# ratt-ru/pfb-clean

Hardware: AMD Instinct MI355X
Metric: PCG matvecs/sec (FFT-conv A^H A apply), 4k x 4k x 8-band cube (higher is better)
Workload: dtype f32; 1 GPU; 4096x4096x8-band cube PCG (hessian_psf + Tikhonov, M = x/sigmainv, tol=0, minit=maxit=20); nx_psf=8192, bands_per_gpu=8, parallelism=band-shard x1, allreduce_hook=False

## Files before the change

pfb_clean_amd/csrc/fftconv_pow2.hip:

```cpp
#include "conv_plan.hpp"
#include "fft_pow2.hpp"
#include <vector>
#include <cstdlib>
#include <type_traits>

namespace pfb {

#ifndef PFB_STAMP
#define PFB_STAMP 0
#endif
#if PFB_STAMP
#define PFB_STAMP_ITS 4
#define PFB_STAMP_FIRST 2
static __device__ unsigned long long* g_stamp_buf = nullptr;
#define STAMP(KID, it, slot)                                                                              \
    do {                                                                                                  \
        const unsigned _si = (unsigned)((it) - PFB_STAMP_FIRST);                                          \
        if (threadIdx.x == 0 && g_stamp_buf && _si < PFB_STAMP_ITS && blockIdx.x < 1024)                  \
            g_stamp_buf[(((size_t)(KID) * 1024 + blockIdx.x) * PFB_STAMP_ITS + _si) * 16 + (slot)] = wall_clock64(); \
    } while (0)
#else
#define STAMP(KID, it, slot) do { (void)(it); } while (0)
#endif

// ... 787 lines not shown
    if constexpr (K < NREG) {
        hook(PassIdx<K>{});
        Blk<T, NVB> o;
#pragma unroll
        for (int h = 0; h < NVB; ++h) {
            cplx<T> w;
            if constexpr (P::BIG) w = K == 0 ? lw[h] : lw[h] * root32<T>(P::KR * K);
            else w = lw[MS * K + h];
            if (PAR) w = w * wq1;
            const cplx<T> zv = za[h][F::cpad(MS * K)];
            cplx<T> zm = zb[h][F::cpad(MS * (NREG - 1 - K))];
            if constexpr (PAR == 0 && K == 0) { if (first0 && h == 0) zm = zv; }
            o.c[h] = T(0.5) * addrot<false>(addc(zv, zm), w * subc(zv, zm));
        }
        storeb<T, NVB>(ub + (size_t)K * ustep + voff, o);
        __builtin_amdgcn_sched_barrier(0);
        post_steps_lin<T, L, PAR, K + 1, NREG, Hook>(za, zb, lw, wq1, ub, ustep, voff, first0, hook);
    }
}

template <typename T, int L, int PAR, typename Hook = NoPassHook>
__device__ __forceinline__ void fwdp_post(const cplx<T>* zr, const cplx<T>* ltm, cplx<T> wq1,
                                          cplx<T>* __restrict__ Tb, int nx, int i0, int rr, int bi,
                                          const Hook& hook = Hook()) {
    using P = FwdP<T, L>;
    using F = typename P::F;
    constexpr int NVB = P::NVB, BS = P::BSTEP, MS = NVB * BS;
    constexpr int NBP = PAR ? P::NBO : P::NBE;
    constexpr int NIT = (NBP + BS - 1) / BS;
    constexpr int NREG = PAR ? NIT : NIT - 1;
    static_assert(MS % 16 == 0, "a step keeps the padding phase");
    static_assert(PAR ? (NBP == NIT * BS) : (NBP == (NIT - 1) * BS + 1), "block counts of the two sweeps");
    cplx<T>* ub = Tb + (size_t)(PAR ? P::NBE : 0) * nx * NVB;
    const size_t ustep = (size_t)BS * nx * NVB;
    const unsigned voff = ((unsigned)bi * (unsigned)nx + (unsigned)(i0 + rr)) * NVB;
    const int m0 = NVB * bi;
    const cplx<T>* za[NVB];
    const cplx<T>* zb[NVB];
#pragma unroll
    for (int h = 0; h < NVB; ++h) {
        za[h] = zr + F::pad(m0 + h);
        zb[h] = zr + F::pad(L - PAR - (m0 + h) - MS * (NREG - 1));
    }
    post_steps_lin<T, L, PAR, 0, NREG, Hook>(za, zb, ltm + m0, wq1, ub, ustep, voff, bi == 0, hook);
    if constexpr (PAR == 0) {
        hook(PassIdx<NREG>{});
        const cplx<T> z0 = zr[F::pad(0)];
        Blk<T, NVB> o;
        o.c[0] = T(0.5) * addrot<false>(addc(z0, z0), cplx<T>(T(-1), T(0)) * subc(z0, z0));
#pragma unroll
        for (int h = 1; h < NVB; ++h) o.c[h] = cplx<T>(0, 0);
        storeb<T, NVB>(ub + (size_t)(NBP - 1) * nx * NVB + (unsigned)(i0 + rr) * NVB, o);
        __builtin_amdgcn_sched_barrier(0);
    }
}

template <typename T, int L, bool BEAM>
__global__ void __launch_bounds__((FwdP<T, L>::NT))
k_row_fwd_pow2q(const T* __restrict__ x, const T* __restrict__ beam, cplx<T>* __restrict__ Tw, const cplx<T>* __restrict__ twM,
                const cplx<T>* __restrict__ ptwc, FastDims d, int band0, int tiles_per_band, int ntiles,
                cplx<T> wq1) {
    using P = FwdP<T, L>;
    constexpr int E = P::E;
    using F = RegFft<T, L, E, false, 0, true, false>;
    constexpr int TPB = F::TPB, G = P::G, NT = P::NT, NP = F::NPASS;
    using V2 = typename vec2<T>::type;
    extern __shared__ __attribute__((aligned(16))) char smem[];
    cplx<T>* ltw = reinterpret_cast<cplx<T>*>(smem);
    cplx<T>* ltm = ltw + P::PTWP;
    cplx<T>* lds0 = ltm + P::NTM;
    int vb = blockIdx.x;
    if (vb >= ntiles) return;
    for (int k = threadIdx.x; k < F::PTWC; k += NT) ltw[k] = ptwc[k];
    for (int k = threadIdx.x; k < P::NTM; k += NT) ltm[k] = twM[k];
    V2 xa[E], ba[BEAM ? E : 1];
    {
        const int bl = vb / tiles_per_band, i0 = P::tile_row(vb - bl * tiles_per_band, tiles_per_band);
        const int g = threadIdx.x / TPB, t = threadIdx.x % TPB;
        const size_t off = (size_t)bl * d.xband + (size_t)(i0 + g) * d.xpitch;
        const V2* xr = reinterpret_cast<const V2*>(x + off) + t;
#pragma unroll
        for (int j = 0; j < E; ++j) xa[j] = xr[TPB * j];
        if constexpr (BEAM) {
            const V2* br = reinterpret_cast<const V2*>(beam + off) + t;
#pragma unroll
            for (int j = 0; j < E; ++j) ba[j] = br[TPB * j];
        }
    }
    __syncthreads();
    for (int sit = 0;; ++sit) {
        STAMP(0, sit, 0);
        const int vbn = vb + (int)gridDim.x < ntiles ? vb + (int)gridDim.x : vb;
        const int bl = vb / tiles_per_band, i0 = P::tile_row(vb - bl * tiles_per_band, tiles_per_band);
        cplx<T>* Tb = Tw + (size_t)(band0 + bl) * d.T_band;
        cplx<T> vv[E];
        {
            const int tid = launder((int)threadIdx.x);
            const int g = tid / TPB, t = tid % TPB;
            cplx<T>* lds = lds0 + (size_t)g * P::STRIDE;
#pragma unroll
            for (int j = 0; j < E; ++j) {
                if constexpr (BEAM) { xa[j].x *= ba[j].x; xa[j].y *= ba[j].y; }
                vv[j] = cplx<T>(xa[j].x, xa[j].y);
            }
            STAMP(0, sit, 1);
            F::template run<false>(vv, lds, t, ltw);
            STAMP(0, sit, 2);
        }
        {
            const int tid = launder((int)threadIdx.x);
            const int g = tid / TPB, t = tid % TPB;
            __syncthreads();
            cplx<T>* wp = lds0 + (size_t)g * P::STRIDE + F::pad(t);
#pragma unroll
            for (int j = 0; j < E; ++j) wp[F::cpad(TPB * j)] = vv[j];
            __syncthreads();
        }
        STAMP(0, sit, 3);
        {
            const int tid = launder((int)threadIdx.x);
            fwdp_post<T, L, 0>(lds0 + (size_t)(tid % G) * P::STRIDE, ltm, wq1, Tb, d.nx, i0, tid % G, tid / G);
        }
        STAMP(0, sit, 4);
        {
            const int tid = launder((int)threadIdx.x);
            const int g = tid / TPB, t = tid % TPB;
            cplx<T>* lds = lds0 + (size_t)g * P::STRIDE;
#pragma unroll
            for (int j = 0; j < E; ++j) {
                vv[j] = cplx<T>(xa[j].x, xa[j].y) * P::tw_row(ltm, t, j);
                if ((j & 3) == 3) __builtin_amdgcn_sched_barrier(0);
            }
            const int bln = vbn / tiles_per_band, i0n = P::tile_row(vbn - bln * tiles_per_band, tiles_per_band);
            const size_t offn = (size_t)bln * d.xband + (size_t)(i0n + g) * d.xpitch;
            const V2* xr = reinterpret_cast<const V2*>(x + offn) + t;
            const V2* br = BEAM ? reinterpret_cast<const V2*>(beam + offn) + t : nullptr;
            F::template run<false>(vv, lds, t, ltw, [&](auto k) {
                constexpr int K = decltype(k)::value;
#pragma unroll
                for (int j = (K * E) / NP; j < ((K + 1) * E) / NP; ++j) {
                    xa[j] = xr[TPB * j];
                    if constexpr (BEAM) ba[j] = br[TPB * j];
                }
            });
            STAMP(0, sit, 5);
        }
        {
            const int tid = launder((int)threadIdx.x);
            const int g = tid / TPB, t = tid % TPB;
            cplx<T>* wp = lds0 + (size_t)g * P::STRIDE + F::pad(t);
            __syncthreads();
#pragma unroll
            for (int j = 0; j < E; ++j) wp[F::cpad(TPB * j)] = vv[j];
            __syncthreads();
            fwdp_post<T, L, 1>(lds0 + (size_t)(tid % G) * P::STRIDE, ltm, wq1, Tb, d.nx, i0, tid % G, tid / G);
            STAMP(0, sit, 6);
            __syncthreads();
        }
        STAMP(0, sit, 7);
        if (vbn == vb) break;
        vb = vbn;
    }
}

template <typename T, int L, int E, int PAR, typename PF>
__device__ __forceinline__ void row_inv_phase(PF&& after_loads_issued, const cplx<T>* __restrict__ Tb,
                                              const cplx<T>* __restrict__ twQ,
                                              const cplx<T>* __restrict__ ptw, cplx<T>* lds0,
                                              cplx<T>* lds, int nx, int i0, int t,
                                              cplx<T> (&vv)[E]) {
    using F = RegFft<T, L, E, RowCfg<T, L, true>::WAVE, InvDb<T, L>::OFF, true>;
    constexpr int TPB = F::TPB;
    constexpr int G = row_groups<T, L, E, RowCfg<T, L, true>::GMAX>();
    constexpr int NT = G * TPB;
    constexpr int STRIDE = F::LDS_ELEMS + 4;
    const int rr = threadIdx.x % G, bi = threadIdx.x / G;
    cplx<T>* yr = lds0 + (size_t)rr * STRIDE;
    __syncthreads();
    constexpr int NVB = FastCfg<T>::NVB;
    constexpr int NBE = nblocks_even(L, NVB);
    constexpr int NBP = PAR ? nblocks_odd(L, NVB) : NBE;
    constexpr int BSTEP = NT / G;
    const cplx<T>* Tp = Tb + ((size_t)(PAR ? NBE : 0) * nx + i0 + rr) * NVB;
    constexpr int NIT = (NBP + BSTEP - 1) / BSTEP;
    Blk<T, NVB> y[NIT];
#pragma unroll
    for (int k = 0; k < NIT; ++k) {
        const int b = bi + k * BSTEP;
        if (b < NBP) y[k] = loadb<T, NVB>(Tp + (size_t)b * nx * NVB);
    }
    after_loads_issued();
#pragma unroll
    for (int k = 0; k < NIT; ++k) {
        const int b = bi + k * BSTEP;
        if (b < NBP) {
#pragma unroll
            for (int h = 0; h < NVB; ++h)
                if (PAR || NVB * b + h <= L) yr[F::pad(NVB * b + h)] = y[k].c[h];
        }
    }
    __syncthreads();
#pragma unroll
    for (int j = 0; j < E; ++j) {
        const int m = t + TPB * j;
        cplx<T> yv = lds[F::pad(m)];
        cplx<T> ym = lds[F::pad(PAR ? (L - 1 - m) : (L - m))];
        if (!PAR && m == 0) { yv.y = 0; ym.y = 0; }
        const cplx<T> w = twQ[2 * m + PAR];
        vv[j] = addrot<true>(addc(yv, ym), mulc(subc(yv, ym), w));
        if ((j & 3) == 3) __builtin_amdgcn_sched_barrier(0);
    }
    F::template run<true>(vv, lds, t, ptw);
}

template <typename T, int L, int E>
__global__ void __launch_bounds__((row_groups<T, L, E, RowCfg<T, L, true>::GMAX>() * (L / E)))
k_row_inv_pow2(const cplx<T>* __restrict__ Tw, const cplx<T>* __restrict__ twQ,
               const cplx<T>* __restrict__ twM, const cplx<T>* __restrict__ ptw,
               const T* __restrict__ x, const T* __restrict__ beam,
               const T* __restrict__ dot_with, const T* __restrict__ dot_with2, T* __restrict__ out,
               double* __restrict__ partials, FastDims d, int band0, T scale, T sigmainv) {
    using F = RegFft<T, L, E, RowCfg<T, L, true>::WAVE, InvDb<T, L>::OFF, true>;
    constexpr int TPB = F::TPB;
    constexpr int G = row_groups<T, L, E, RowCfg<T, L, true>::GMAX>();
    constexpr int NT = G * TPB;
    constexpr int STRIDE = F::LDS_ELEMS + 4;
    constexpr int HP = G / 2;
    using V2 = typename vec2<T>::type;
    extern __shared__ __attribute__((aligned(16))) char smem[];
    double* red = reinterpret_cast<double*>(smem);
    cplx<T>* ltw = reinterpret_cast<cplx<T>*>(smem + 384);
    cplx<T>* lds0 = ltw + ((F::PTWC + 1) & ~1);
    const int g = threadIdx.x / TPB, t = threadIdx.x % TPB;
    cplx<T>* lds = lds0 + (size_t)g * STRIDE;
    for (int k = threadIdx.x; k < F::PTWC; k += NT) ltw[k] = ptw[k];
    const int rg = xcd_row_group<G>(blockIdx.x, gridDim.x);
    const int i0 = rg * G;
    const int bl = blockIdx.y, band = band0 + bl;
    const cplx<T>* Tb = Tw + (size_t)band * d.T_band;
    cplx<T> vv[E], ev[E];
    row_inv_phase<T, L, E, 0>([] {}, Tb, twQ, ltw, lds0, lds, d.nx, i0, t, ev);
    const size_t rowoff = ((size_t)bl * d.nx + (i0 + g)) * d.ny;
    const V2* xr = reinterpret_cast<const V2*>(x + rowoff) + t;
    const V2* br = beam ? reinterpret_cast<const V2*>(beam + rowoff) + t : nullptr;
    const V2* dr = dot_with ? reinterpret_cast<const V2*>(dot_with + rowoff) + t : nullptr;
    const V2* dr2 = dot_with2 ? reinterpret_cast<const V2*>(dot_with2 + rowoff) + t : nullptr;
    V2* orow = reinterpret_cast<V2*>(out + rowoff) + t;
    const bool dot_is_x = dot_with == x;
    constexpr bool BIG32 = sizeof(T) == 4 && E >= 16 && L >= 4096;
    constexpr bool MIXBIG = odd_part(L) > 1 && (NT >= 1024 || E >= 16 || (sizeof(T) == 8 && NT >= 512));
    constexpr bool PREF = !BIG32 && !MIXBIG && (sizeof(T) == 4 || NT < 1024);
    V2 xq[PREF ? E : 1], rq[PREF ? E : 1];
    row_inv_phase<T, L, E, 1>([&] {
        if constexpr (PREF) {
#pragma unroll
            for (int j = 0; j < E; ++j) {
                xq[j] = xr[TPB * j];
                if (dr2) rq[j] = dr2[TPB * j];
            }
        }
    }, Tb, twQ, ltw, lds0, lds, d.nx, i0, t, vv);
    double acc[3] = {0.0, 0.0, 0.0};
    const cplx<T>* tm = twM + t;
#pragma unroll
    for (int j = 0; j < E; ++j) {
        const cplx<T> zz = ev[j] + mulc(vv[j], tm[TPB * j]);
        V2 val;
        val.x = zz.x * scale;
        val.y = zz.y * scale;
        if (br) { const V2 b = br[TPB * j]; val.x *= b.x; val.y *= b.y; }
        V2 xx;
        if constexpr (PREF) xx = xq[j]; else xx = xr[TPB * j];
        val.x += sigmainv * xx.x;
        val.y += sigmainv * xx.y;
        orow[TPB * j] = val;
        if (dr) {
            V2 dw = xx;
            if (!dot_is_x) dw = dr[TPB * j];
            acc[0] += (double)dw.x * (double)val.x + (double)dw.y * (double)val.y;
            if (dr2) {
                V2 d2;
                if constexpr (PREF) d2 = rq[j]; else d2 = dr2[TPB * j];
                acc[1] += (double)d2.x * (double)val.x + (double)d2.y * (double)val.y;
            }
            acc[2] += (double)val.x * (double)val.x + (double)val.y * (double)val.y;
        }
    }
    if (dot_with) {
        __syncthreads();
        block_sum<3>(acc, red);
        if (threadIdx.x == 0) {
            const size_t np = (size_t)gridDim.x * gridDim.y, k = (size_t)bl * gridDim.x + rg;
            partials[k] = acc[0]; partials[np + k] = acc[1]; partials[2 * np + k] = acc[2];
        }
    }
}

constexpr int INV_ROT = 3;
constexpr int INV_HOIST_B = 8;
template <typename T, int L, int E>
struct InvP {
    using C = RowCfg<T, L, true>;
    using F = RegFft<T, L, E, C::WAVE, 0, true>;
    static constexpr bool PARK = sizeof(T) == 4 && E < 16;
    static constexpr int G = (sizeof(T) == 4 ? 1024 : 512) / F::TPB;
    static constexpr int NT = G * F::TPB;
    static constexpr int STRIDE = F::LDS_ELEMS + 4;
    static constexpr int NVB = FastCfg<T>::NVB;
    static constexpr int NBE = nblocks_even(L, NVB);
    static constexpr int NBO = nblocks_odd(L, NVB);
    static constexpr int BSTEP = NT / G;
    static constexpr int NITE = (NBE + BSTEP - 1) / BSTEP;
    static constexpr int NITO = (NBO + BSTEP - 1) / BSTEP;
    static constexpr int PTWP = (F::PTWC + 1) & ~1;
    static constexpr bool SMT = E >= 16;
    static constexpr bool OPF = E < 16;
    static constexpr bool NXT = OPF || sizeof(T) == 8;
    static constexpr bool NXE = !NXT;
    static constexpr int NTM = SMT ? F::TPB : L;
    static constexpr size_t LDS = 384 + sizeof(cplx<T>) * ((size_t)PTWP + NTM + (size_t)G * STRIDE + (PARK ? (size_t)G * L : 0));
    static constexpr bool OK = odd_part(L) == 1 && LDS <= (size_t)LDS_MAX && !C::WAVE && (!SMT || 32 * F::TPB == 2 * L) &&
                               (sizeof(T) == 4 ? (NT == 1024 && G >= 4 && G <= 16) : (NT == 512 && (G == 2 || G == 4) && L >= 1024));
    __device__ __forceinline__ static cplx<T> tw_row(const cplx<T>* ltm, int t, int j) {
        if constexpr (SMT) return j == 0 ? ltm[t] : ltm[t] * root32<T>(j);
        else return ltm[t + F::TPB * j];
    }
};

template <typename T, int L> struct InvPE {
    static constexpr int MINL64 = 4096;
    static constexpr int E = (sizeof(T) == 8 && L >= MINL64) ? 16 : RowCfg<T, L, true>::E;
};

template <typename T, int L>
constexpr bool invp_class(int e, bool park, bool opf, bool smt, bool nxt) {
    using P = InvP<T, L, InvPE<T, L>::E>;
    return P::OK && InvPE<T, L>::E == e && P::PARK == park && P::OPF == opf && P::SMT == smt && P::NXT == nxt &&
           P::NXE == !nxt && P::SMT == !opf && (nxt || sizeof(T) == 4);
}
static_assert(invp_class<float, 1024>(8, true, true, false, true) && invp_class<float, 2048>(8, true, true, false, true));
static_assert(invp_class<double, 1024>(8, false, true, false, true) && invp_class<double, 2048>(8, false, true, false, true));
static_assert(invp_class<double, 4096>(16, false, false, true, true) && invp_class<float, 4096>(16, false, false, true, false));

template <typename T, int L, int E>
constexpr bool inv_pb_ok() { return odd_part(L) == 1 && !(sizeof(T) == 4 && InvP<T, L, E>::SMT); }

template <typename T, int L, int E>
constexpr bool inv_lin_ok() {
    using P = InvP<T, L, E>;
    return sizeof(T) == 4 && P::NBO % P::BSTEP == 0 && P::NBE == P::NBO + 1 && P::NITO * P::BSTEP == P::NBO &&
           P::NITE == P::NITO + 1 && (P::NVB * P::BSTEP) % 16 == 0 && P::F::TPB % 16 == 0;
}
template <typename T, int L, int E, int PAR, int K0, int K1>
__device__ __forceinline__ void inv_issue_slice(const cplx<T>* __restrict__ Tb, int nx, int i0, int rr, int bi,
                                                Blk<T, FastCfg<T>::NVB> (&y)[InvP<T, L, E>::NITE]);
template <typename T, int L, int E, int PAR>
__device__ __forceinline__ void inv_issue(const cplx<T>* __restrict__ Tb, int nx, int i0, int rr, int bi,
                                          Blk<T, FastCfg<T>::NVB> (&y)[InvP<T, L, E>::NITE]) {
    using P = InvP<T, L, E>;
    constexpr int NBP = PAR ? P::NBO : P::NBE, NIT = PAR ? P::NITO : P::NITE;
    if constexpr (inv_lin_ok<T, L, E>()) {
        inv_issue_slice<T, L, E, PAR, 0, NIT>(Tb, nx, i0, rr, bi, y);
        return;
    }
    const cplx<T>* Tp = Tb + ((size_t)(PAR ? P::NBE : 0) * nx + i0 + rr) * P::NVB;
#pragma unroll
    for (int k = 0; k < NIT; ++k) {
        int b = bi + k * P::BSTEP;
        if (b >= NBP) b = NBP - 1;
        y[k] = loadb<T, P::NVB>(Tp + (size_t)b * nx * P::NVB);
    }
}

template <typename T, int L, int E, int PAR, int K0, int K1>
__device__ __forceinline__ void inv_issue_slice(const cplx<T>* __restrict__ Tb, int nx, int i0, int rr, int bi,
                                                Blk<T, FastCfg<T>::NVB> (&y)[InvP<T, L, E>::NITE]) {
    using P = InvP<T, L, E>;
    constexpr int NBP = PAR ? P::NBO : P::NBE;
    if constexpr (inv_lin_ok<T, L, E>()) {
        const cplx<T>* ub = Tb + (size_t)(PAR ? P::NBE : 0) * nx * P::NVB;
        const size_t ustep = (size_t)P::BSTEP * nx * P::NVB;
        const unsigned vrow = (unsigned)(i0 + rr) * P::NVB, voff = (unsigned)bi * (unsigned)nx * P::NVB + vrow;
#pragma unroll
        for (int k = K0; k < K1; ++k) {
            if (PAR == 0 && k == P::NITE - 1) y[k] = loadb<T, P::NVB>(ub + (size_t)(NBP - 1) * nx * P::NVB + vrow);
            else y[k] = loadb<T, P::NVB>(ub + (size_t)k * ustep + voff);
        }
        return;
    }
    const cplx<T>* Tp = Tb + ((size_t)(PAR ? P::NBE : 0) * nx + i0 + rr) * P::NVB;
#pragma unroll
    for (int k = K0; k < K1; ++k) {
        int b = bi + k * P::BSTEP;
        if (b >= NBP) b = NBP - 1;
        y[k] = loadb<T, P::NVB>(Tp + (size_t)b * nx * P::NVB);
    }
}

template <typename T, int L, int E, int PAR>
__device__ __forceinline__ void inv_scatter(const Blk<T, FastCfg<T>::NVB> (&y)[InvP<T, L, E>::NITE],
                                            cplx<T>* yr, int bi) {
    using P = InvP<T, L, E>;
    constexpr int NBP = PAR ? P::NBO : P::NBE, NIT = PAR ? P::NITO : P::NITE;
    if constexpr (inv_lin_ok<T, L, E>()) {
        cplx<T>* y0 = yr + P::F::pad(P::NVB * bi);
#pragma unroll
        for (int k = 0; k < NIT; ++k) {
            if (PAR == 0 && k == NIT - 1) yr[P::F::pad(L)] = y[k].c[0];
            else {
#pragma unroll
                for (int h = 0; h < P::NVB; ++h) y0[P::F::cpad(P::NVB * P::BSTEP * k) + h] = y[k].c[h];
            }
        }
        return;
    }
#pragma unroll
    for (int k = 0; k < NIT; ++k) {
        int b = bi + k * P::BSTEP;
        if (b >= NBP) b = NBP - 1;
#pragma unroll
        for (int h = 0; h < P::NVB; ++h)
            if (PAR || P::NVB * b + h <= L) yr[P::F::pad(P::NVB * b + h)] = y[k].c[h];
    }
}

template <typename T, int L, int E, int PAR>
__device__ __forceinline__ void inv_build(const cplx<T>* lds, const cplx<T>* ltm, cplx<T> wq1, int t,
                                          cplx<T> (&vv)[E]) {
    using F = typename InvP<T, L, E>::F;
    if constexpr (inv_lin_ok<T, L, E>()) {
        const cplx<T>* pa = lds + F::pad(t);
        const cplx<T>* pb = lds + F::pad(L - PAR - t - F::TPB * (E - 1));
#pragma unroll
        for (int j = 0; j < E; ++j) {
            cplx<T> yv = pa[F::cpad(F::TPB * j)];
            cplx<T> ym = pb[F::cpad(F::TPB * (E - 1 - j))];
            if (!PAR && j == 0) { if (t == 0) { yv.y = 0; ym.y = 0; } }
            cplx<T> w = InvP<T, L, E>::tw_row(ltm, t, j);
            if (PAR) w = w * wq1;
            vv[j] = addrot<true>(addc(yv, ym), mulc(subc(yv, ym), w));
            if ((j & 3) == 3) __builtin_amdgcn_sched_barrier(0);
        }
        return;
    }
#pragma unroll
    for (int j = 0; j < E; ++j) {
        const int m = t + F::TPB * j;
        cplx<T> yv = lds[F::pad(m)];
        cplx<T> ym = lds[F::pad(PAR ? (L - 1 - m) : (L - m))];
        if (!PAR && m == 0) { yv.y = 0; ym.y = 0; }
        cplx<T> w = InvP<T, L, E>::tw_row(ltm, t, j);
        if (PAR) w = w * wq1;
        vv[j] = addrot<true>(addc(yv, ym), mulc(subc(yv, ym), w));
        if ((j & 3) == 3) __builtin_amdgcn_sched_barrier(0);
    }
}

template <typename T, int L, int E, int MODE, bool BEAM, bool PB = false>
__global__ void __launch_bounds__((InvP<T, L, E>::NT), (InvP<T, L, E>::NT / 256))
k_row_inv_pow2p(const cplx<T>* __restrict__ Tw, const cplx<T>* __restrict__ twM,
                const cplx<T>* __restrict__ ptw, const T* __restrict__ x, const T* __restrict__ beam,
                const T* __restrict__ dot_with2, T* __restrict__ out,
                double* __restrict__ partials, FastDims d, int band0, int tiles_per_band, int ntiles,
                T scale, T sigmainv, cplx<T> wq1) {
    using P = InvP<T, L, E>;
    using F = typename P::F;
    constexpr int TPB = F::TPB, G = P::G, NT = P::NT;
    constexpr bool BATCH = P::NXE && !(BEAM && MODE == 2);
    constexpr int NP = F::NPASS, NPA = NP / 2 > 0 ? NP / 2 : 1, NPB = NP - NPA > 0 ? NP - NPA : 1;
    using V2 = typename vec2<T>::type;
    extern __shared__ __attribute__((aligned(16))) char smem[];
    double* red = reinterpret_cast<double*>(smem);
    cplx<T>* ltw = reinterpret_cast<cplx<T>*>(smem + 384);
    cplx<T>* ltm = ltw + P::PTWP;
    cplx<T>* lds0 = ltm + P::NTM;
    cplx<T>* park = lds0 + (size_t)G * P::STRIDE;
    int vb = blockIdx.x;
    if (vb >= ntiles) return;
    for (int k = threadIdx.x; k < F::PTWC; k += NT) ltw[k] = ptw[k];
    for (int k = threadIdx.x; k < P::NTM; k += NT) ltm[k] = twM[k];
    constexpr int SH = 128 / (G * (int)sizeof(cplx<T>) * P::NVB) > 1 ? 128 / (G * (int)sizeof(cplx<T>) * P::NVB) : 1;
    const bool pairing = SH > 1 && (tiles_per_band % (8 * SH)) == 0;
    auto tile = [&](int v, int& bl, int& i0) {
        bl = v / tiles_per_band;
        int rg = v - bl * tiles_per_band;
        if (pairing) rg = xcd_paired(rg, SH);
        i0 = rg * G;
    };
    int bl, i0;
    tile(vb, bl, i0);
    Blk<T, P::NVB> y[P::NITE];
    if constexpr (P::NXT || BATCH)
        inv_issue<T, L, E, 0>(Tw + (size_t)(band0 + bl) * d.T_band, d.nx, i0, threadIdx.x % G, threadIdx.x / G, y);
    double acc[3] = {0.0, 0.0, 0.0};
    if constexpr (PB && MODE >= 1) {
        if (threadIdx.x == 0) {
            const int n = 3 * (ntiles / tiles_per_band);
            for (int k = 0; k < n; ++k) partials[(size_t)k * gridDim.x + blockIdx.x] = 0.0;
        }
    }
    V2 ov[P::PARK ? E : 1];
    V2* oprev = nullptr;
    for (int sit = 0;; ++sit) {
        STAMP(2, sit, 0);
        const int s1 = sit + 1;
        const int cand = (int)(((unsigned)blockIdx.x + (unsigned)s1 * (unsigned)INV_ROT) % gridDim.x) + s1 * (int)gridDim.x;
        const int vbn = cand < ntiles ? cand : vb;
        int bln, i0n;
        tile(vbn, bln, i0n);
        const cplx<T>* Tb = Tw + (size_t)(band0 + bl) * d.T_band;
        if constexpr (!P::NXT && !BATCH) {
            const int tid = launder((int)threadIdx.x);
            inv_issue<T, L, E, 0>(Tb, d.nx, i0, tid % G, tid / G, y);
        }
        cplx<T> vv[E], ev[P::PARK ? 1 : E];
        constexpr bool OPF = P::OPF;
        V2 xq[OPF ? E : 1], rq[(OPF && MODE == 2) ? E : 1], bq[(OPF && BEAM) ? E : 1];
        {
            const int tid = launder((int)threadIdx.x);
            const int g = tid / TPB, t = tid % TPB, rr = tid % G, bi = tid / G;
            cplx<T>* lds = lds0 + (size_t)g * P::STRIDE;
            if (!P::NXT || sit == 0) __syncthreads();
            STAMP(2, sit, 1);
            inv_scatter<T, L, E, 0>(y, lds0 + (size_t)rr * P::STRIDE, bi);
            STAMP(2, sit, 2);
            inv_issue_slice<T, L, E, 1, 0, P::NITO / NPA>(Tb, d.nx, i0, rr, bi, y);
            __syncthreads();
            STAMP(2, sit, 3);
            inv_build<T, L, E, 0>(lds, ltm, wq1, t, vv);
            STAMP(2, sit, 4);
            {
                const size_t rowoff = ((size_t)bl * d.nx + (i0 + g)) * d.ny;
                const V2* xr = reinterpret_cast<const V2*>(x + rowoff) + t;
                const V2* br = BEAM ? reinterpret_cast<const V2*>(beam + rowoff) + t : nullptr;
                F::template run<true>(vv, lds, t, ltw, [&](auto k) {
                    constexpr int K = decltype(k)::value;
                    if constexpr (P::PARK) {
                        if (oprev) {
#pragma unroll
                            for (int j = (K * E) / NP; j < ((K + 1) * E) / NP; ++j) oprev[TPB * j] = ov[j];
                        }
                    }
                    if constexpr (K < NPA) {
                        if constexpr (K != 0)
                        inv_issue_slice<T, L, E, 1, (K * P::NITO) / NPA, ((K + 1) * P::NITO) / NPA>(Tb, d.nx, i0, rr, bi, y);
                    } else if constexpr (OPF) {
                        constexpr int KK = K - NPA;
#pragma unroll
                        for (int j = (KK * E) / NPB; j < ((KK + 1) * E) / NPB; ++j) {
                            xq[j] = xr[TPB * j];
                            if constexpr (BEAM) bq[j] = br[TPB * j];
                        }
                    }
                });
            }
            STAMP(2, sit, 5);
#pragma unroll
            for (int j = 0; j < E; ++j) {
                if constexpr (P::PARK) park[j * NT + tid] = vv[j]; else ev[j] = vv[j];
            }
        }
        {
            const int tid = launder((int)threadIdx.x);
            const int g = tid / TPB, t = tid % TPB, rr = tid % G, bi = tid / G;
            cplx<T>* lds = lds0 + (size_t)g * P::STRIDE;
            __syncthreads();
            STAMP(2, sit, 6);
            inv_scatter<T, L, E, 1>(y, lds0 + (size_t)rr * P::STRIDE, bi);
            STAMP(2, sit, 7);
            const size_t rowoff = ((size_t)bl * d.nx + (i0 + g)) * d.ny;
            const V2* dr2 = reinterpret_cast<const V2*>(dot_with2 + rowoff) + t;
            const cplx<T>* Tbn = Tw + (size_t)(band0 + bln) * d.T_band;
            if constexpr (MODE == 2 && OPF) {
#pragma unroll
                for (int j = 0; j < E / NPA; ++j) rq[j] = dr2[TPB * j];
            }
            __syncthreads();
            STAMP(2, sit, 8);
            inv_build<T, L, E, 1>(lds, ltm, wq1, t, vv);
            STAMP(2, sit, 9);
            F::template run<true>(vv, lds, t, ltw, [&](auto k) {
                constexpr int K = decltype(k)::value;
                if constexpr (MODE == 2 && OPF) {
                    if constexpr (K < NPA) {
                        if constexpr (K != 0)
#pragma unroll
                        for (int j = (K * E) / NPA; j < ((K + 1) * E) / NPA; ++j) rq[j] = dr2[TPB * j];
                    } else {
                        constexpr int KK = K - NPA;
                        inv_issue_slice<T, L, E, 0, (KK * P::NITE) / NPB, ((KK + 1) * P::NITE) / NPB>(Tbn, d.nx, i0n, rr, bi, y);
                    }
                } else if constexpr (P::NXT) {
                    inv_issue_slice<T, L, E, 0, (K * P::NITE) / NP, ((K + 1) * P::NITE) / NP>(Tbn, d.nx, i0n, rr, bi, y);
                }
            });
            STAMP(2, sit, 10);
            if constexpr (P::NXT) __syncthreads();
        }
        {
            const int tid = launder((int)threadIdx.x);
            int g = tid / TPB;
            const int t = tid % TPB;
            if constexpr (TPB % 64 == 0 && !P::OPF) g = __builtin_amdgcn_readfirstlane(g);
            const size_t rowoff = ((size_t)bl * d.nx + (i0 + g)) * d.ny;
            V2* orow = reinterpret_cast<V2*>(out + rowoff) + t;
            [[maybe_unused]] const V2* xr_e = reinterpret_cast<const V2*>(x + rowoff) + t;
            [[maybe_unused]] const V2* br_e = BEAM ? reinterpret_cast<const V2*>(beam + rowoff) + t : nullptr;
            [[maybe_unused]] const V2* dr_e = MODE == 2 ? reinterpret_cast<const V2*>(dot_with2 + rowoff) + t : nullptr;
            if constexpr (!OPF) {
#pragma unroll
                for (int j = 0; j < E; ++j) vv[j] = ev[j] + mulc(vv[j], P::tw_row(ltm, t, j));
                __builtin_amdgcn_sched_barrier(0);
            }
            [[maybe_unused]] V2 xh[BATCH ? E : 1], rh[(BATCH && MODE == 2) ? E : 1], bh[(BATCH && BEAM) ? E : 1];

#pragma unroll
            for (int j = 0; j < E; ++j) {
                cplx<T> zz;
                if constexpr (!OPF) zz = vv[j];
                else {
                    cplx<T> e0;
                    if constexpr (P::PARK) e0 = park[j * NT + tid]; else e0 = ev[j];
                    zz = e0 + mulc(vv[j], P::tw_row(ltm, t, j));
                }
                if constexpr (BATCH) {
                    constexpr int HB = INV_HOIST_B;
                    if (j % HB == 0) {
                        __builtin_amdgcn_sched_barrier(0);
#pragma unroll
                        for (int q = j; q < j + HB && q < E; ++q) {
                            xh[q] = xr_e[TPB * q];
                            if constexpr (MODE == 2) rh[q] = dr_e[TPB * q];
                            if constexpr (BEAM) bh[q] = br_e[TPB * q];
                        }
                        if (j + HB >= E)
                            inv_issue<T, L, E, 0>(Tw + (size_t)(band0 + bln) * d.T_band, d.nx, i0n, tid % G, tid / G, y);
                        __builtin_amdgcn_sched_barrier(0);
                    }
                }
                V2 val;
                V2 xx;
                [[maybe_unused]] V2 bb;
                if constexpr (OPF) { xx = xq[j]; if constexpr (BEAM) bb = bq[j]; }
                else if constexpr (BATCH) { xx = xh[j]; if constexpr (BEAM) bb = bh[j]; }
                else { xx = xr_e[TPB * j]; if constexpr (BEAM) bb = br_e[TPB * j]; }
                if constexpr (BEAM) {
                    val.x = zz.x * scale * bb.x + sigmainv * xx.x;
                    val.y = zz.y * scale * bb.y + sigmainv * xx.y;
                } else {
                    val.x = zz.x * scale + sigmainv * xx.x;
                    val.y = zz.y * scale + sigmainv * xx.y;
                }
                if constexpr (P::PARK) ov[j] = val; else orow[TPB * j] = val;
                if constexpr (!OPF && !BATCH) { if (sizeof(T) == 4 && (j & 3) == 3) __builtin_amdgcn_sched_barrier(0); }
                if constexpr (MODE >= 1) {
                    acc[0] += (double)xx.x * (double)val.x + (double)xx.y * (double)val.y;
                    if constexpr (MODE == 2) {
                        V2 d2;
                        if constexpr (OPF) d2 = rq[j]; else if constexpr (BATCH) d2 = rh[j];
                        else d2 = dr_e[TPB * j];
                        acc[1] += (double)d2.x * (double)val.x + (double)d2.y * (double)val.y;
                    }
                    acc[2] += (double)val.x * (double)val.x + (double)val.y * (double)val.y;
                }
            }
        }
        STAMP(2, sit, 11);
        if constexpr (P::PARK) {
            const int tid = launder((int)threadIdx.x);
            const int g = tid / TPB, t = tid % TPB;
            oprev = reinterpret_cast<V2*>(out + ((size_t)bl * d.nx + (i0 + g)) * d.ny) + t;
        }
        if constexpr (PB && MODE >= 1) {
            if (vbn == vb || bln != bl) {
                block_sum<3>(acc, red);
                if (threadIdx.x == 0) {
                    const size_t np = (size_t)(ntiles / tiles_per_band) * gridDim.x, k = (size_t)bl * gridDim.x + blockIdx.x;
                    partials[k] = acc[0]; partials[np + k] = acc[1]; partials[2 * np + k] = acc[2];
                }
                acc[0] = 0.0; acc[1] = 0.0; acc[2] = 0.0;
            }
        }
        if (vbn == vb) break;
        vb = vbn; bl = bln; i0 = i0n;
    }
    if constexpr (P::PARK) {
        if (oprev) {
#pragma unroll
            for (int j = 0; j < E; ++j) oprev[TPB * j] = ov[j];
        }
    }
    if constexpr (!PB && MODE >= 1) {
        __syncthreads();
        block_sum<3>(acc, red);
        if (threadIdx.x == 0) {
            const size_t np = gridDim.x;
            partials[blockIdx.x] = acc[0]; partials[np + blockIdx.x] = acc[1]; partials[2 * np + blockIdx.x] = acc[2];
        }
    }
}


template <typename Fn>
static inline bool for_pow2_size(int n, Fn&& f) {
    switch (n) {
#define X(NN) case NN: f(std::integral_constant<int, NN>{}); return true;
        X(64) X(128) X(256) X(512) X(1024) X(2048) X(4096) X(8192)
#undef X
        default: return false;
    }
}

template <typename Fn>
static inline bool for_mix_size(int n, Fn&& f) {
    switch (n) {
#define X(NN) case NN: f(std::integral_constant<int, NN>{}); return true;
        X(96) X(192) X(384) X(768) X(1536) X(3072) X(6144)
        X(80) X(160) X(320) X(640) X(1280) X(2560) X(5120)
#undef X
        default: return false;
    }
}
constexpr int MIX_COL_MIN = 96, MIX_ROW_MIN = 80;
constexpr int mix_row_max(bool f32) { return f32 ? 6144 : 3072; }
inline bool mix_len(int n, int lo, int hi) { return (odd_part(n) == 3 || odd_part(n) == 5) && n >= lo && n <= hi; }
inline bool mix_col_len(int nx) { return mix_len(nx, MIX_COL_MIN, 6144); }
inline bool mix_row_len(int L, bool f32) { return mix_len(L, MIX_ROW_MIN, mix_row_max(f32)); }
constexpr int ROW_TILE_MAX = 32;

constexpr bool col_two_level(int nx) { return odd_part(nx) == 1 && nx >= 8192; }

enum Tab {
    PTW_COL,
    PTWC_COL,
    PTW_ROW,
    PTWC_ROW_FWD,
    PTWC_ROW_INV,
    PTWC_ROW_INV_P,
    TW_M,
    NTAB
};
struct FastTables {
    void* tab[NTAB];
    int num_cu;
};

struct ColPass {
    int (*prepare)(pfb_conv_plan* p, FastTables* ft);
    int (*launch)(pfb_conv_plan* p, const FastTables* ft, int band0, int nb, hipStream_t st);
    int (*fwd_launch)(pfb_conv_plan* p, const FastTables* ft, const void* Tq, int band, hipStream_t st);
};
struct RowPass {
    int (*prepare)(pfb_conv_plan* p, FastTables* ft);
    int (*rows_per_wg)(const pfb_conv_plan* p);
    int (*fwd_launch)(pfb_conv_plan* p, const FastTables* ft, void* Tbuf, int band0, int nb, const void* x,
                      const void* beam, size_t xpitch, size_t xband, hipStream_t st);
    int (*inv_launch)(pfb_conv_plan* p, const FastTables* ft, const ApplyArgs& a);
};
const ColPass& col_pass_pow2();
const RowPass& row_pass_pow2();
const ColPass& col_pass_mix();
const RowPass& row_pass_mix();
inline const ColPass& col_pass(const pfb_conv_plan* p) { return mix_col_len(p->nx) ? col_pass_mix() : col_pass_pow2(); }
inline const RowPass& row_pass(const pfb_conv_plan* p) {
    return mix_row_len(p->ny / 2, p->dtype == PFB_F32) ? row_pass_mix() : row_pass_pow2();
}
static int unsupported_len(const char* axis, int n) {
    set_error("pow2: unsupported %s %d", axis, n);
    return PFB_ERR_UNSUPPORTED;
}

template <typename T, typename Fill>
static int upload_table(void** dev, int n, Fill&& fill) {
    std::vector<cplx<T>> h(n > 0 ? n : 1);
    if (n > 0) fill(h.data());
    PFB_HIP_CHECK(hipMalloc(dev, sizeof(cplx<T>) * h.size()));
    PFB_HIP_CHECK(hipMemcpy(*dev, h.data(), sizeof(cplx<T>) * h.size(), hipMemcpyHostToDevice));
    return PFB_OK;
}
template <typename T, int N, int E>
static int upload_ptw(void** dev) { return upload_table<T>(dev, ptw_total<N, E>(), fill_ptw<T, N, E>); }
template <typename T, int N, int E>
static int upload_ptwc(void** dev) { return upload_table<T>(dev, ptw_total<N, E>() / 4, fill_ptw_compact<T, N, E>); }

template <typename K>
static int set_lds_max(K* kernel) {
    PFB_HIP_CHECK(hipFuncSetAttribute((const void*)kernel, hipFuncAttributeMaxDynamicSharedMemorySize, LDS_MAX));
    return PFB_OK;
}

static inline int balanced_grid(int need, int maxgrid) {
    if (need <= maxgrid) return need;
    const int trips = (need + maxgrid - 1) / maxgrid;
    return (need + trips - 1) / trips;
}

enum class ColKind { Plain, Persistent, TwoLevel };
constexpr int col_resident(int threads) { return (8 * 64) / threads > 0 ? (8 * 64) / threads : 1; }
template <typename T, int H> struct ColCfg {
    static constexpr int NVB = FastCfg<T>::NVB;
    static constexpr int E1 = ecol<T, H>();
    using F1 = RegFft<T, H, E1>;
    static constexpr int GC1 = col_groups<H, E1>(), NT1 = GC1 * F1::TPB;
    static constexpr size_t XB1 = sizeof(cplx<T>) * (size_t)GC1 * NVB * F1::LDS_ELEMS;
    static constexpr size_t TAB1 = sizeof(cplx<T>) * (size_t)((F1::PTWC + 1) & ~1);
    static constexpr ColKind KIND = odd_part(H) > 1 ? ColKind::Plain : col_two_level(H) ? ColKind::TwoLevel
                                  : H >= 2048 && XB1 + TAB1 <= (size_t)LDS_MAX ? ColKind::Persistent : ColKind::Plain;
    static constexpr bool DB = KIND == ColKind::Persistent && col_resident(NT1) == 1 && 2 * XB1 + TAB1 <= (size_t)LDS_MAX;

    struct Shape { int gc, threads; size_t lds; int wg_per_cu, tab_n, tab_e; };
    static constexpr Shape shape() {
        if constexpr (KIND == ColKind::TwoLevel) {
            using CX = ColX<T, H, ECOLX>;
            const int wg_lds = (int)((size_t)LDS_MAX / CX::LDS);
            int wg_per_cu = col_resident(CX::NT);
            if (wg_per_cu > wg_lds) wg_per_cu = wg_lds > 0 ? wg_lds : 1;
            return {CX::GC, CX::NT, CX::LDS, wg_per_cu, CX::HS, ECOLX};
        } else if constexpr (KIND == ColKind::Persistent) {
            return {GC1, NT1, (DB ? 2 : 1) * XB1 + TAB1, col_resident(NT1), H, E1};
        } else {
            return {GC1, NT1, XB1, 0, H, E1};
        }
    }
};

template <typename T, int H> struct ColKernels {
    using C = ColCfg<T, H>;
    static constexpr auto plain() { return k_col_pow2<T, H, C::E1>; }
    static constexpr auto fwd() { return k_col_fwd_pow2<T, H, C::E1>; }
    template <typename Fn> static void serving(Fn&& f) {
        if constexpr (C::KIND == ColKind::Persistent) {
            f(k_col_pow2p<T, H, C::E1, C::DB, false>, false);
            f(k_col_pow2p<T, H, C::E1, C::DB, true>, true);
        } else if constexpr (C::KIND == ColKind::TwoLevel) {
            f(k_col_pow2x<T, H, ECOLX, false>, false);
            f(k_col_pow2x<T, H, ECOLX, true>, true);
        }
    }
    template <typename Fn> static void all(Fn&& f) {
        if constexpr (C::KIND == ColKind::Plain) f(plain());
        f(fwd());
        serving([&](auto* k, bool) { f(k); });
        if constexpr (H == 4096 && sizeof(T) == 8) {
            f(k_col_pow2x<T, H, ECOLX, false>);
            f(k_col_pow2x<T, H, ECOLX, true>);
        }
    }
};

template <typename T, int H>
static int launch_col(pfb_conv_plan* p, const FastTables* ft, int band0, int nb, hipStream_t st) {
    using C = ColCfg<T, H>;
    using CK = ColKernels<T, H>;
    constexpr auto S = C::shape();
    const int nblk = fast_nblocks(p->ny / 2, FastCfg<T>::NVB);
    if constexpr (C::KIND == ColKind::Plain) {
        hipLaunchKernelGGL(CK::plain(), dim3((nblk + S.gc - 1) / S.gc, nb), dim3(S.threads), S.lds, st,
                           (cplx<T>*)p->T, (const cplx<T>*)p->psf_l, (const cplx<T>*)p->twP,
                           (const cplx<T>*)ft->tab[PTW_COL], nblk, p->T_elems_per_band, p->psf_elems_per_band, band0);
    } else {
        const int band_first = band0 + nb - 1;
        const bool psf_nt = sizeof(cplx<T>) * p->psf_elems_per_band * (size_t)nb >= ((size_t)200 << 20);
        const int nitems = nblk * nb, need = (nitems + S.gc - 1) / S.gc, maxgrid = ft->num_cu * S.wg_per_cu;
        const int grid = C::KIND == ColKind::Persistent ? balanced_grid(need, maxgrid) : (need < maxgrid ? need : maxgrid);
        CK::serving([&](auto* k, bool nt) {
            if (nt != psf_nt) return;
            hipLaunchKernelGGL(k, dim3(grid), dim3(S.threads), S.lds, st,
                               (cplx<T>*)p->T, (const cplx<T>*)p->psf_l, (const cplx<T>*)p->twP,
                               (const cplx<T>*)ft->tab[PTWC_COL], nblk, nitems, p->T_elems_per_band,
                               p->psf_elems_per_band, band_first, -1);
        });
    }
    return PFB_OK;
}

template <typename T, int H>
static int launch_col_fwd(pfb_conv_plan* p, const FastTables* ft, const void* Tq, int band, hipStream_t st) {
    using C = ColCfg<T, H>;
    using CK = ColKernels<T, H>;
    const int L = p->ny / 2;
    const int nblk = fast_nblocks(L, C::NVB), nbe = nblocks_even(L, C::NVB);
    hipLaunchKernelGGL(CK::fwd(), dim3((nblk + C::GC1 - 1) / C::GC1), dim3(C::NT1), C::XB1, st,
                       (const cplx<T>*)Tq, (cplx<T>*)p->psf_l + (size_t)band * p->psf_elems_per_band,
                       (const cplx<T>*)p->twP, (const cplx<T>*)ft->tab[PTW_COL], nblk, nbe, p->T_elems_per_band,
                       col_two_level(H));
    return PFB_OK;
}

template <typename T, int H>
static int col_prepare(FastTables* ft) {
    constexpr auto S = ColCfg<T, H>::shape();
    int rc = upload_ptw<T, H, ColCfg<T, H>::E1>(&ft->tab[PTW_COL]);
    if constexpr (ColCfg<T, H>::KIND != ColKind::Plain)
        if (rc == PFB_OK) rc = upload_ptwc<T, S.tab_n, S.tab_e>(&ft->tab[PTWC_COL]);
    ColKernels<T, H>::all([&](auto* k) { if (rc == PFB_OK) rc = set_lds_max(k); });
    return rc;
}

template <typename D> struct ColPassOf {
    static int prepare(pfb_conv_plan* p, FastTables* ft) {
        return D::each(p, [&](auto t, auto h) { return col_prepare<decltype(t), h()>(ft); });
    }
    static int launch(pfb_conv_plan* p, const FastTables* ft, int band0, int nb, hipStream_t st) {
        return D::each(p, [&](auto t, auto h) { return launch_col<decltype(t), h()>(p, ft, band0, nb, st); });
    }
    static int fwd_launch(pfb_conv_plan* p, const FastTables* ft, const void* Tq, int band, hipStream_t st) {
        return D::each(p, [&](auto t, auto h) { return launch_col_fwd<decltype(t), h()>(p, ft, Tq, band, st); });
    }
    static constexpr ColPass table = {prepare, launch, fwd_launch};
};

template <typename T, int L> constexpr bool fwdp_ok() {
    if constexpr (odd_part(L) > 1) return false;
    else return FwdP<T, L>::OK;
}
template <typename T, int L> struct RowFwdK {
    using FP = FwdP<T, L>;
    static constexpr bool PERSISTENT = fwdp_ok<T, L>();
    static constexpr int E = [] { if constexpr (PERSISTENT) return FP::E; else return RowCfg<T, L, false>::E; }();
    static constexpr auto plain() { return k_row_fwd_pow2<T, L, E>; }
    template <typename Fn> static void reachable(Fn&& f) {
        if constexpr (PERSISTENT) {
            f(k_row_fwd_pow2q<T, L, false>, false);
            f(k_row_fwd_pow2q<T, L, true>, true);
        } else {
            f(plain(), false);
        }
    }
};

template <typename T, int L> struct RowInvK {
    static constexpr int E = RowCfg<T, L, true>::E, EP = InvPE<T, L>::E;
    using IP = InvP<T, L, EP>;
    static constexpr bool PERSISTENT = IP::OK;
    static constexpr bool PER_BAND = PERSISTENT && inv_pb_ok<T, L, EP>();
    static constexpr auto plain() { return k_row_inv_pow2<T, L, E>; }
    template <int MODE, bool PB, typename Fn> static void beam_pair(Fn&& f) {
        f(k_row_inv_pow2p<T, L, EP, MODE, false, PB>, MODE, false, PB);
        f(k_row_inv_pow2p<T, L, EP, MODE, true, PB>, MODE, true, PB);
    }
    template <typename Fn> static void persistent(Fn&& f) {
        if constexpr (PERSISTENT) {
            beam_pair<0, false>(f);
            beam_pair<1, false>(f);
            beam_pair<2, false>(f);
            if constexpr (PER_BAND) beam_pair<2, true>(f);
        }
    }
    template <typename Fn> static void reachable(Fn&& f) {
        f(plain());
        persistent([&](auto* k, int, bool, bool) { f(k); });
    }
};

template <typename T, int L>
static int row_prepare(FastTables* ft) {
    using FK = RowFwdK<T, L>;
    using IK = RowInvK<T, L>;
    int rc;
    if constexpr (FK::PERSISTENT) rc = upload_ptwc<T, L, FK::E>(&ft->tab[PTWC_ROW_FWD]);
    else rc = upload_ptw<T, L, FK::E>(&ft->tab[PTW_ROW]);
    if (rc == PFB_OK) rc = upload_ptwc<T, L, IK::E>(&ft->tab[PTWC_ROW_INV]);
    if constexpr (IK::EP != IK::E) {
        if (rc == PFB_OK) rc = upload_ptwc<T, L, IK::EP>(&ft->tab[PTWC_ROW_INV_P]);
    } else {
        ft->tab[PTWC_ROW_INV_P] = ft->tab[PTWC_ROW_INV];
    }
    FK::reachable([&](auto* k, bool) { if (rc == PFB_OK) rc = set_lds_max(k); });
    IK::reachable([&](auto* k) { if (rc == PFB_OK) rc = set_lds_max(k); });
    return rc;
}

template <typename T, int L>
static int rows_per_wg() { return row_groups<T, L, RowCfg<T, L, true>::E, RowCfg<T, L, true>::GMAX>(); }

static FastDims fast_dims(const pfb_conv_plan* p, size_t xpitch, size_t xband) {
    return FastDims{p->nx, p->ny, p->M, p->T_elems_per_band, p->psf_elems_per_band, xpitch, xband};
}
template <typename T>
static cplx<T> wq1_of(const pfb_conv_plan* p) {
    const long double a = 6.283185307179586476925286766559005768L / (2.0L * (long double)p->ny);
    return cplx<T>((T)cosl(a), (T)(-sinl(a)));
}

template <typename T, int L>
static int launch_row_fwd(pfb_conv_plan* p, const FastTables* ft, void* Tbuf, int band0, int nb, const void* x,
                          const void* beam, size_t xpitch, size_t xband, hipStream_t st) {
    using K = RowFwdK<T, L>;
    const FastDims d = fast_dims(p, xpitch, xband);
// ... 290 lines not shown
```

Measured before the change: 429.3 cube-matvecs/s.

## Land next tile's even bins in a second LDS set during odd-pass FFT

```diff
diff --git a/pfb_clean_amd/csrc/fftconv_pow2.hip b/pfb_clean_amd/csrc/fftconv_pow2.hip
--- a/pfb_clean_amd/csrc/fftconv_pow2.hip
+++ b/pfb_clean_amd/csrc/fftconv_pow2.hip
@@ -1113,7 +1113,8 @@
 struct InvP {
     using C = RowCfg<T, L, true>;
     using F = RegFft<T, L, E, C::WAVE, 0, true>;
-    static constexpr bool PARK = sizeof(T) == 4 && E < 16;
+    static constexpr bool LAND2 = sizeof(T) == 4 && E < 16;
+    static constexpr bool DST = LAND2;
     static constexpr int G = (sizeof(T) == 4 ? 1024 : 512) / F::TPB;
     static constexpr int NT = G * F::TPB;
     static constexpr int STRIDE = F::LDS_ELEMS + 4;
@@ -1126,11 +1127,12 @@
     static constexpr int PTWP = (F::PTWC + 1) & ~1;
     static constexpr bool SMT = E >= 16;
     static constexpr bool OPF = E < 16;
-    static constexpr bool NXT = OPF || sizeof(T) == 8;
-    static constexpr bool NXE = !NXT;
+    static constexpr bool NXT = sizeof(T) == 8;
+    static constexpr bool NXE = !NXT && !LAND2;
     static constexpr int NTM = SMT ? F::TPB : L;
-    static constexpr size_t LDS = 384 + sizeof(cplx<T>) * ((size_t)PTWP + NTM + (size_t)G * STRIDE + (PARK ? (size_t)G * L : 0));
-    static constexpr bool OK = odd_part(L) == 1 && LDS <= (size_t)LDS_MAX && !C::WAVE && (!SMT || 32 * F::TPB == 2 * L) &&
+    static constexpr int LROT = 16 / G > 2 ? 16 / G : 2;
+    __device__ __forceinline__ static int land_at(int m, int r) { return (m + r * LROT) & (L - 1); }
+    static constexpr size_t LDS = 384 + sizeof(cplx<T>) * ((size_t)PTWP + NTM + (size_t)G * STRIDE + (LAND2 ? (size_t)G * L : 0));    static constexpr bool OK = odd_part(L) == 1 && LDS <= (size_t)LDS_MAX && !C::WAVE && (!SMT || 32 * F::TPB == 2 * L) &&
                                (sizeof(T) == 4 ? (NT == 1024 && G >= 4 && G <= 16) : (NT == 512 && (G == 2 || G == 4) && L >= 1024));
     __device__ __forceinline__ static cplx<T> tw_row(const cplx<T>* ltm, int t, int j) {
         if constexpr (SMT) return j == 0 ? ltm[t] : ltm[t] * root32<T>(j);
@@ -1144,14 +1146,16 @@
 };
 
 template <typename T, int L>
-constexpr bool invp_class(int e, bool park, bool opf, bool smt, bool nxt) {
+constexpr bool invp_class(int e, bool land2, bool opf, bool smt, bool nxt) {
     using P = InvP<T, L, InvPE<T, L>::E>;
-    return P::OK && InvPE<T, L>::E == e && P::PARK == park && P::OPF == opf && P::SMT == smt && P::NXT == nxt &&
-           P::NXE == !nxt && P::SMT == !opf && (nxt || sizeof(T) == 4);
-}
-static_assert(invp_class<float, 1024>(8, true, true, false, true) && invp_class<float, 2048>(8, true, true, false, true));
+    return P::OK && InvPE<T, L>::E == e && P::LAND2 == land2 && P::DST == land2 && P::OPF == opf && P::SMT == smt &&
+           P::NXT == nxt && P::NXE == (!nxt && !land2) && P::SMT == !opf && !(nxt && land2) && (nxt || sizeof(T) == 4);
+}
+static_assert(invp_class<float, 1024>(8, true, true, false, false) && invp_class<float, 2048>(8, true, true, false, false));
 static_assert(invp_class<double, 1024>(8, false, true, false, true) && invp_class<double, 2048>(8, false, true, false, true));
 static_assert(invp_class<double, 4096>(16, false, false, true, true) && invp_class<float, 4096>(16, false, false, true, false));
+static_assert(InvP<float, 1024, 8>::LDS <= (size_t)LDS_MAX && InvP<float, 2048, 8>::LDS <= (size_t)LDS_MAX, "both landing sets fit the LDS");
+static_assert(InvP<float, 2048, 8>::F::NPASS >= 2 && InvP<float, 1024, 8>::F::NPASS >= 2, "LAND2: request passes, then scatter passes");
 
 template <typename T, int L, int E>
 constexpr bool inv_pb_ok() { return odd_part(L) == 1 && !(sizeof(T) == 4 && InvP<T, L, E>::SMT); }
@@ -1208,15 +1212,30 @@
     }
 }
 
-template <typename T, int L, int E, int PAR>
-__device__ __forceinline__ void inv_scatter(const Blk<T, FastCfg<T>::NVB> (&y)[InvP<T, L, E>::NITE],
-                                            cplx<T>* yr, int bi) {
+template <typename T, int L, int E, int PAR, int K0, int K1, bool FLAT = false>
+__device__ __forceinline__ void inv_scatter_slice(const Blk<T, FastCfg<T>::NVB> (&y)[InvP<T, L, E>::NITE],
+                                                  cplx<T>* yr, int bi, int r = 0, cplx<T>* nyq = nullptr) {
     using P = InvP<T, L, E>;
     constexpr int NBP = PAR ? P::NBO : P::NBE, NIT = PAR ? P::NITO : P::NITE;
+    static_assert(!FLAT || (PAR == 0 && P::NVB % 2 == 0 && P::LROT % P::NVB == 0), "the second landing set: even bins, whole blocks");
+    if constexpr (FLAT) {
+#pragma unroll
+        for (int k = K0; k < K1; ++k) {
+            int b = bi + k * P::BSTEP;
+            if (b >= NBP) b = NBP - 1;
+            if (inv_lin_ok<T, L, E>() ? k == NIT - 1 : P::NVB * b >= L) *nyq = y[k].c[0];
+            else {
+                cplx<T>* y0 = yr + P::land_at(P::NVB * b, r);
+#pragma unroll
+                for (int h = 0; h < P::NVB; ++h) y0[h] = y[k].c[h];
+            }
+        }
+        return;
+    }
     if constexpr (inv_lin_ok<T, L, E>()) {
         cplx<T>* y0 = yr + P::F::pad(P::NVB * bi);
 #pragma unroll
-        for (int k = 0; k < NIT; ++k) {
+        for (int k = K0; k < K1; ++k) {
             if (PAR == 0 && k == NIT - 1) yr[P::F::pad(L)] = y[k].c[0];
             else {
 #pragma unroll
@@ -1226,7 +1245,7 @@
         return;
     }
 #pragma unroll
-    for (int k = 0; k < NIT; ++k) {
+    for (int k = K0; k < K1; ++k) {
         int b = bi + k * P::BSTEP;
         if (b >= NBP) b = NBP - 1;
 #pragma unroll
@@ -1234,11 +1253,30 @@
             if (PAR || P::NVB * b + h <= L) yr[P::F::pad(P::NVB * b + h)] = y[k].c[h];
     }
 }
-
-template <typename T, int L, int E, int PAR>
+template <typename T, int L, int E, int PAR, bool FLAT = false>
+__device__ __forceinline__ void inv_scatter(const Blk<T, FastCfg<T>::NVB> (&y)[InvP<T, L, E>::NITE],
+                                            cplx<T>* yr, int bi, int r = 0, cplx<T>* nyq = nullptr) {
+    inv_scatter_slice<T, L, E, PAR, 0, PAR ? InvP<T, L, E>::NITO : InvP<T, L, E>::NITE, FLAT>(y, yr, bi, r, nyq);
+}
+
+template <typename T, int L, int E, int PAR, bool FLAT = false>
 __device__ __forceinline__ void inv_build(const cplx<T>* lds, const cplx<T>* ltm, cplx<T> wq1, int t,
-                                          cplx<T> (&vv)[E]) {
+                                          cplx<T> (&vv)[E], int r = 0, const cplx<T>* nyq = nullptr) {
     using F = typename InvP<T, L, E>::F;
+    static_assert(!FLAT || PAR == 0, "the second landing set holds even bins");
+    if constexpr (FLAT) {
+#pragma unroll
+        for (int j = 0; j < E; ++j) {
+            const int m = t + F::TPB * j;
+            cplx<T> yv = lds[InvP<T, L, E>::land_at(m, r)];
+            cplx<T> ym = (j == 0 && t == 0) ? *nyq : lds[InvP<T, L, E>::land_at(L - m, r)];
+            if (j == 0) { if (t == 0) { yv.y = 0; ym.y = 0; } }
+            cplx<T> w = InvP<T, L, E>::tw_row(ltm, t, j);
+            vv[j] = addrot<true>(addc(yv, ym), mulc(subc(yv, ym), w));
+            if ((j & 3) == 3) __builtin_amdgcn_sched_barrier(0);
+        }
+        return;
+    }
     if constexpr (inv_lin_ok<T, L, E>()) {
         const cplx<T>* pa = lds + F::pad(t);
         const cplx<T>* pb = lds + F::pad(L - PAR - t - F::TPB * (E - 1));
@@ -1285,7 +1323,7 @@
     cplx<T>* ltw = reinterpret_cast<cplx<T>*>(smem + 384);
     cplx<T>* ltm = ltw + P::PTWP;
     cplx<T>* lds0 = ltm + P::NTM;
-    cplx<T>* park = lds0 + (size_t)G * P::STRIDE;
+    [[maybe_unused]] cplx<T>* land = lds0 + (size_t)G * P::STRIDE;
     int vb = blockIdx.x;
     if (vb >= ntiles) return;
     for (int k = threadIdx.x; k < F::PTWC; k += NT) ltw[k] = ptw[k];
@@ -1301,8 +1339,11 @@
     int bl, i0;
     tile(vb, bl, i0);
     Blk<T, P::NVB> y[P::NITE];
-    if constexpr (P::NXT || BATCH)
+    if constexpr (P::NXT || P::LAND2 || BATCH)
         inv_issue<T, L, E, 0>(Tw + (size_t)(band0 + bl) * d.T_band, d.nx, i0, threadIdx.x % G, threadIdx.x / G, y);
+    if constexpr (P::LAND2)
+        inv_scatter<T, L, E, 0, true>(y, land + (size_t)(threadIdx.x % G) * L, threadIdx.x / G, threadIdx.x % G,
+                                      lds0 + (size_t)(threadIdx.x % G) * P::STRIDE + F::LDS_ELEMS);
     double acc[3] = {0.0, 0.0, 0.0};
     if constexpr (PB && MODE >= 1) {
         if (threadIdx.x == 0) {
@@ -1310,7 +1351,7 @@
             for (int k = 0; k < n; ++k) partials[(size_t)k * gridDim.x + blockIdx.x] = 0.0;
         }
     }
-    V2 ov[P::PARK ? E : 1];
+    V2 ov[P::DST ? E : 1];
     V2* oprev = nullptr;
     for (int sit = 0;; ++sit) {
         STAMP(2, sit, 0);
@@ -1320,25 +1361,28 @@
         int bln, i0n;
         tile(vbn, bln, i0n);
         const cplx<T>* Tb = Tw + (size_t)(band0 + bl) * d.T_band;
-        if constexpr (!P::NXT && !BATCH) {
+        if constexpr (!P::NXT && !P::LAND2 && !BATCH) {
             const int tid = launder((int)threadIdx.x);
             inv_issue<T, L, E, 0>(Tb, d.nx, i0, tid % G, tid / G, y);
         }
-        cplx<T> vv[E], ev[P::PARK ? 1 : E];
+        cplx<T> vv[E], ev[E];
         constexpr bool OPF = P::OPF;
         V2 xq[OPF ? E : 1], rq[(OPF && MODE == 2) ? E : 1], bq[(OPF && BEAM) ? E : 1];
         {
             const int tid = launder((int)threadIdx.x);
             const int g = tid / TPB, t = tid % TPB, rr = tid % G, bi = tid / G;
             cplx<T>* lds = lds0 + (size_t)g * P::STRIDE;
-            if (!P::NXT || sit == 0) __syncthreads();
+            if constexpr (!P::LAND2) {
+                if (!P::NXT || sit == 0) __syncthreads();
+            }
             STAMP(2, sit, 1);
-            inv_scatter<T, L, E, 0>(y, lds0 + (size_t)rr * P::STRIDE, bi);
+            if constexpr (!P::LAND2) inv_scatter<T, L, E, 0>(y, lds0 + (size_t)rr * P::STRIDE, bi);
             STAMP(2, sit, 2);
             inv_issue_slice<T, L, E, 1, 0, P::NITO / NPA>(Tb, d.nx, i0, rr, bi, y);
             __syncthreads();
             STAMP(2, sit, 3);
-            inv_build<T, L, E, 0>(lds, ltm, wq1, t, vv);
+            if constexpr (P::LAND2) inv_build<T, L, E, 0, true>(land + (size_t)g * L, ltm, wq1, t, vv, g, lds + F::LDS_ELEMS);
+            else inv_build<T, L, E, 0>(lds, ltm, wq1, t, vv);
             STAMP(2, sit, 4);
             {
                 const size_t rowoff = ((size_t)bl * d.nx + (i0 + g)) * d.ny;
@@ -1346,7 +1390,7 @@
                 const V2* br = BEAM ? reinterpret_cast<const V2*>(beam + rowoff) + t : nullptr;
                 F::template run<true>(vv, lds, t, ltw, [&](auto k) {
                     constexpr int K = decltype(k)::value;
-                    if constexpr (P::PARK) {
+                    if constexpr (P::DST) {
                         if (oprev) {
 #pragma unroll
                             for (int j = (K * E) / NP; j < ((K + 1) * E) / NP; ++j) oprev[TPB * j] = ov[j];
@@ -1367,9 +1411,7 @@
             }
             STAMP(2, sit, 5);
 #pragma unroll
-            for (int j = 0; j < E; ++j) {
-                if constexpr (P::PARK) park[j * NT + tid] = vv[j]; else ev[j] = vv[j];
-            }
+            for (int j = 0; j < E; ++j) ev[j] = vv[j];
         }
         {
             const int tid = launder((int)threadIdx.x);
@@ -1382,7 +1424,11 @@
             const size_t rowoff = ((size_t)bl * d.nx + (i0 + g)) * d.ny;
             const V2* dr2 = reinterpret_cast<const V2*>(dot_with2 + rowoff) + t;
             const cplx<T>* Tbn = Tw + (size_t)(band0 + bln) * d.T_band;
-            if constexpr (MODE == 2 && OPF) {
+            [[maybe_unused]] cplx<T>* lnd = land + (size_t)rr * L;
+            [[maybe_unused]] cplx<T>* nyq = lds0 + (size_t)rr * P::STRIDE + F::LDS_ELEMS;
+            if constexpr (P::LAND2) {
+                inv_issue_slice<T, L, E, 0, 0, P::NITE / NPA>(Tbn, d.nx, i0n, rr, bi, y);
+            } else if constexpr (MODE == 2 && OPF) {
 #pragma unroll
                 for (int j = 0; j < E / NPA; ++j) rq[j] = dr2[TPB * j];
             }
@@ -1392,6 +1438,21 @@
             STAMP(2, sit, 9);
             F::template run<true>(vv, lds, t, ltw, [&](auto k) {
                 constexpr int K = decltype(k)::value;
+                if constexpr (P::LAND2) {
+                    if constexpr (K < NPA) {
+                        if constexpr (K != 0)
+                        inv_issue_slice<T, L, E, 0, (K * P::NITE) / NPA, ((K + 1) * P::NITE) / NPA>(Tbn, d.nx, i0n, rr, bi, y);
+                    } else {
+                        constexpr int KK = K - NPA;
+                        if constexpr (MODE == 2) {
+#pragma unroll
+                            for (int j = (KK * E) / NPB; j < ((KK + 1) * E) / NPB; ++j) rq[j] = dr2[TPB * j];
+                            __builtin_amdgcn_sched_barrier(0);
+                        }
+                        if constexpr (KK < NPA)
+                            inv_scatter_slice<T, L, E, 0, (KK * P::NITE) / NPA, ((KK + 1) * P::NITE) / NPA, true>(y, lnd, bi, rr, nyq);
+                    }
+                } else
                 if constexpr (MODE == 2 && OPF) {
                     if constexpr (K < NPA) {
                         if constexpr (K != 0)
@@ -1430,9 +1491,7 @@
                 cplx<T> zz;
                 if constexpr (!OPF) zz = vv[j];
                 else {
-                    cplx<T> e0;
-                    if constexpr (P::PARK) e0 = park[j * NT + tid]; else e0 = ev[j];
-                    zz = e0 + mulc(vv[j], P::tw_row(ltm, t, j));
+                    zz = ev[j] + mulc(vv[j], P::tw_row(ltm, t, j));
                 }
                 if constexpr (BATCH) {
                     constexpr int HB = INV_HOIST_B;
@@ -1462,7 +1521,7 @@
                     val.x = zz.x * scale + sigmainv * xx.x;
                     val.y = zz.y * scale + sigmainv * xx.y;
                 }
-                if constexpr (P::PARK) ov[j] = val; else orow[TPB * j] = val;
+                if constexpr (P::DST) ov[j] = val; else orow[TPB * j] = val;
                 if constexpr (!OPF && !BATCH) { if (sizeof(T) == 4 && (j & 3) == 3) __builtin_amdgcn_sched_barrier(0); }
                 if constexpr (MODE >= 1) {
                     acc[0] += (double)xx.x * (double)val.x + (double)xx.y * (double)val.y;
@@ -1477,7 +1536,7 @@
             }
         }
         STAMP(2, sit, 11);
-        if constexpr (P::PARK) {
+        if constexpr (P::DST) {
             const int tid = launder((int)threadIdx.x);
             const int g = tid / TPB, t = tid % TPB;
             oprev = reinterpret_cast<V2*>(out + ((size_t)bl * d.nx + (i0 + g)) * d.ny) + t;
@@ -1495,7 +1554,7 @@
         if (vbn == vb) break;
         vb = vbn; bl = bln; i0 = i0n;
     }
-    if constexpr (P::PARK) {
+    if constexpr (P::DST) {
         if (oprev) {
 #pragma unroll
             for (int j = 0; j < E; ++j) oprev[TPB * j] = ov[j];
```

Result: no change. 430.8 cube-matvecs/s (median of 4 runs) (+0.3%).
